# Healthcare-Robotics/assistive-gym

Measured on AMD Instinct MI355X. Metric: env_steps_per_sec, higher is better.
Workload: dtype f32; 1 GPU; FeedingJaco-v1, 4096 lockstep envs per MI355X, random-policy rollout, 5 simulation steps per env step, 50 PGS sweeps; envs_per_gpu=4096, global_envs=4096, reset_pool=256, reset=pool, parallelism=env-sharded x1, obs_allgather=False

## Files before the change

__graft_entry__.py:

```python
import os
import subprocess
import sys

ROOT = os.path.dirname(os.path.abspath(__file__))
if ROOT not in sys.path:
    sys.path.insert(0, ROOT)


def build():
    from assistive_gym_amd.build import build as build_lib
    build_lib(force=True)
    build_lib(out=os.path.join(ROOT, 'assistive_gym_amd', 'lib', 'variants', 'lvs.so'), extra=('-DAGX_PGS_LV=3',), only=['FEEDING'])
    build_lib(out=os.path.join(ROOT, 'assistive_gym_amd', 'lib', 'variants', 'solo.so'), extra=('-DAGX_SOLVE_PAIR=0',), only=['FEEDING'])
    build_lib(out=os.path.join(ROOT, 'assistive_gym_amd', 'lib', 'variants', 'scan4.so'), extra=('-DAGX_GJK_SCAN_WIDE=0', '-DAGX_GJK_SCAN_ONE=0'), only=['FEEDING'])
    build_lib(out=os.path.join(ROOT, 'assistive_gym_amd', 'lib', 'variants', 'finishgjk.so'), extra=('-DAGX_FINISH_SPILL_GJK',), only=['FEEDING'])
    build_lib(out=os.path.join(ROOT, 'assistive_gym_amd', 'lib', 'variants', 'faceplain.so'), extra=('-DAGX_FACE_PLAIN',), only=['FEEDING', 'FEEDING_M'])
    subprocess.check_call(['make', '-C', os.path.join(ROOT, 'oracle')], stdout=subprocess.DEVNULL)
    if os.path.isdir('/root/reference/assistive_gym/envs/assets'):
        from assistive_gym_amd.model import compiler
        compiler.main()
    import assistive_gym_amd
    from assistive_gym_amd import libagx
    L = libagx.load()
    missing = [e for e in libagx.EXPORTS if not hasattr(L, e)]
    assert not missing, missing


def smoke():
    import numpy as np
    sys.path.insert(0, os.path.join(ROOT, 'tests'))
    from assistive_gym_amd import libagx
    from assistive_gym_amd.blob import ModelBlob
    from assistive_gym_amd.vec_env import build_reset_pool
    from oracle_lib import Oracle
    libagx.check(libagx.load().agx_selftest(0), 'agx_selftest')
    n = 64
    for model in ('feeding_jaco', 'bed_bathing_sawyer'):
        blob = ModelBlob.load(model)
        states = build_reset_pool(blob, n, seed=1001)
        st = libagx.Stepper(blob, n)
        st.set_state(states)
        actions = np.random.RandomState(0).uniform(-1, 1, (n, blob.act_dim)).astype(np.float32)
        obs, rew, done, info = st.step_host(actions)
        o = Oracle(blob)
        worst = 0.0
        for i in range(8):
            o_obs, o_rew, _, o_info = o.step(states[i].copy(), actions[i])
            worst = max(worst, float(np.abs(obs[i] - o_obs).max()), abs(float(rew[i]) - o_rew))
        assert np.isfinite(obs).all() and np.isfinite(rew).all()
        assert worst < 1e-3, (model, worst)
        print('smoke ok: 64 %s envs stepped on the GPU (%s kernels), max |obs, reward| deviation from the oracle %.2e' % (model, st.variant(), worst))
        st.close()


if __name__ == '__main__':
    build()
    if len(sys.argv) > 1 and sys.argv[1] == 'smoke':
        smoke()
```

assistive_gym_amd/csrc/agx_collide.h:

```cpp
#pragma once

namespace agx {

struct Cand { v3 pa, pb, n; float dist, gap; };
constexpr float GJK_FAR_MARGIN = 1e-4f;

AGX_DEV void make_shape(const Ctx& c, int col, v3 shift, gjk_shape& s) {
  s.n = CLI(c, col, AGX_C_NVERT);
  s.v = c.bf + c.o_vert + 3 * CLI(c, col, AGX_C_VOFF);
  v3 p; body_xf(c, CLI(c, col, AGX_C_BODY), s.R, p);
  s.p = p - shift; s.box = false;
  s.c = mul(s.R, mk3(CLF(c, col, AGX_C_AABB_C), CLF(c, col, AGX_C_AABB_C + 1), CLF(c, col, AGX_C_AABB_C + 2))) + s.p;
}
AGX_DEV bool narrowphase(const Ctx& c, int ca, int cb, float limit, Cand& out, bool has) {
  const float* AB = c.lds + L_ARENA;
  gjk_shape sa, sb;
  sa.v = nullptr; sa.n = 0; sa.box = false; sa.c = mk3(0.f, 0.f, 0.f); sb.v = nullptr; sb.n = 0; sb.box = false; sb.c = sa.c;
  v3 shift = mk3(0.f, 0.f, 0.f);
  float ra = 0.f, rb = 0.f;
  bool ok = has;
  if (has) {
    shift = mk3(0.5f * (AB[ABS * ca] + AB[ABS * ca + 3]), 0.5f * (AB[ABS * ca + 1] + AB[ABS * ca + 4]), 0.5f * (AB[ABS * ca + 2] + AB[ABS * ca + 5]));
    make_shape(c, ca, shift, sa); make_shape(c, cb, shift, sb);
    if (CLI(c, cb, AGX_C_BODY) == AGX_BODY_WORLD && sb.n == 8 && (CLI(c, cb, AGX_C_TAG) == AGX_TAG_TABLE || CLI(c, cb, AGX_C_TAG) == AGX_TAG_PLANE)) {
      sb.box = true;
      float lo[3], hi[3];
      for (int k = 0; k < 3; k++) {
        lo[k] = fmaxf(AB[ABS * cb + k], AB[ABS * ca + k] - AGX_BOX_CLIP); hi[k] = fminf(AB[ABS * cb + 3 + k], AB[ABS * ca + 3 + k] + AGX_BOX_CLIP);
        if (hi[k] < lo[k]) ok = false;
      }
      sb.lo = mk3(lo[0], lo[1], lo[2]) - shift; sb.hi = mk3(hi[0], hi[1], hi[2]) - shift; sb.c = 0.5f * (sb.lo + sb.hi);
    }
    ra = CLF(c, ca, AGX_C_RADIUS); rb = CLF(c, cb, AGX_C_RADIUS);
  }
  float d; v3 pa, pb, n;
  const bool pen = gjk_distance(sa, sb, PRM(c, AGX_P_GJK_TOL), (int)PRM(c, AGX_P_GJK_MAXIT), limit + ra + rb + GJK_FAR_MARGIN, ok, d, pa, pb);
  if (!ok) return false;
  if (!pen) {
    if (d - ra - rb >= limit) return false;
    n = (1.0f / d) * (pa - pb);
  } else {
    float depth; gjk_penetration(sa, sb, c.bf + c.o_dirs, c.bi[AGX_H_NDIR], depth, n, pa, pb);
    d = -depth;
  }
  out.pa = pa - ra * n + shift; out.pb = pb + rb * n + shift; out.n = n; out.dist = d - ra - rb;
  return true;
}
AGX_DEV float pair_mu(const Ctx& c, int ca, int cb) {
  float plane_mu = c.lds[L_ST + c.s_env + AGX_E_PLANE_FRICTION];
  float mua = CLI(c, ca, AGX_C_TAG) == AGX_TAG_PLANE ? plane_mu : CLF(c, ca, AGX_C_FRICTION);
  float mub = CLI(c, cb, AGX_C_TAG) == AGX_TAG_PLANE ? plane_mu : CLF(c, cb, AGX_C_FRICTION);
  return mua * mub;
}
AGX_DEV void emit_contact(Ctx& c, int slot, int ca, int cb, const Cand& k) {
  float* o = c.gcon + CON_STRIDE * slot; int* oi = (int*)o;
  oi[C_CA] = ca; oi[C_CB] = cb; oi[C_BA] = CLI(c, ca, AGX_C_BODY); oi[C_BB] = CLI(c, cb, AGX_C_BODY);
  st3(o + C_PA, k.pa); st3(o + C_PB, k.pb); st3(o + C_N, k.n); o[C_DIST] = k.dist; o[C_MU] = pair_mu(c, ca, cb); o[C_LAM] = 0.f;
}
constexpr int CAND_STRIDE = 8;
constexpr int TW_WORDS = 6 * (MAX_DOF + MAX_FREE);
constexpr int WL_FIT = (ARENA_WORDS - ABS * MAX_COLL - TW_WORDS) / (1 + CAND_STRIDE);
constexpr int WL_MAX = WL_FIT < 200 ? WL_FIT : 200;
constexpr int A_WL = ABS * MAX_COLL;
constexpr int WL_KEY_MASK = ~((511 << 9) | (3 << 24));
constexpr int A_CAND = A_WL + WL_MAX;
constexpr int A_TW = A_CAND + WL_MAX * CAND_STRIDE;
static_assert(A_TW + TW_WORDS <= ARENA_WORDS, "collision workspace exceeds the arena");
static_assert(MAX_COLL <= 512, "collider indices are packed in 9 bits");
constexpr bool LIST_BYTES = MAX_COLL <= 256;
constexpr int LIST_TAIL = LIST_BYTES ? 8 : 16;
constexpr int WL_CAP = WL_MAX - LIST_TAIL;
template <bool B> struct ListIndex { typedef unsigned short type; };
template <> struct ListIndex<true> { typedef uint8_t type; };
typedef ListIndex<LIST_BYTES>::type list_t;
static_assert(WL_CAP >= 128, "a flush of at least two full passes");

AGX_DEV void emit_from_cand(Ctx& c, int slot, int idx) {
  const float* L = c.lds; const int pr = c.ldsi[L_ARENA + A_WL + idx]; const float* cd = L + L_ARENA + A_CAND + CAND_STRIDE * idx;
  Cand k; k.gap = cd[0]; k.pa = ld3(cd + 1); k.n = ld3(cd + 4); k.dist = cd[7]; k.pb = k.pa - k.dist * k.n;
  emit_contact(c, slot, pr & 511, (pr >> 9) & 511, k);
}
AGX_DEV bool face_box(const Ctx& c, int cb) {
  return CLI(c, cb, AGX_C_BODY) == AGX_BODY_WORLD && CLI(c, cb, AGX_C_NVERT) == 8 && (CLI(c, cb, AGX_C_TAG) == AGX_TAG_TABLE || CLI(c, cb, AGX_C_TAG) == AGX_TAG_PLANE);
}
AGX_DEV bool face_point(const Ctx& c, int ca, int cb, int e, v3 p0, Cand& out) {
  const float* AB = c.lds + L_ARENA;
  const int n = CLI(c, ca, AGX_C_NVERT);
  const float* V = c.bf + c.o_vert + 3 * CLI(c, ca, AGX_C_VOFF);
  m3 R; v3 p; body_xf(c, CLI(c, ca, AGX_C_BODY), R, p);
  const float x0 = AB[ABS * cb], y0 = AB[ABS * cb + 1], x1 = AB[ABS * cb + 3], y1 = AB[ABS * cb + 4], top = AB[ABS * cb + 5];
  float zmin = 3.0e38f;
  for (int v = 0; v < n; v++) { const v3 w = mul(R, mk3(V[3 * v], V[3 * v + 1], V[3 * v + 2])) + p; if (w.x >= x0 && w.x <= x1 && w.y >= y0 && w.y <= y1 && w.z < zmin) zmin = w.z; }
  float cx[1 + AGX_FACE_EXTRA], cy[1 + AGX_FACE_EXTRA];
  cx[0] = p0.x; cy[0] = p0.y;
#pragma unroll
  for (int q = 1; q <= AGX_FACE_EXTRA; q++) { cx[q] = 0.f; cy[q] = 0.f; }
  v3 pick = mk3(0.f, 0.f, 0.f);
  if (e == 0) {
    bool found = false;
    for (int v = 0; v < n && !found; v++) {
      const v3 w = mul(R, mk3(V[3 * v], V[3 * v + 1], V[3 * v + 2])) + p;
      if (w.x >= x0 && w.x <= x1 && w.y >= y0 && w.y <= y1 && w.z <= zmin + AGX_FACE_BAND) { pick = w; found = true; }
    }
    if (!found) return false;
  }
#pragma unroll
  for (int q = 1; q <= AGX_FACE_EXTRA; q++) {
    if (q > e) break;
    int bi = -1; float bd = AGX_FACE_SPREAD * AGX_FACE_SPREAD; v3 bw = mk3(0.f, 0.f, 0.f);
    for (int v = 0; v < n; v++) {
      const v3 w = mul(R, mk3(V[3 * v], V[3 * v + 1], V[3 * v + 2])) + p;
      if (!(w.x >= x0 && w.x <= x1 && w.y >= y0 && w.y <= y1) || w.z > zmin + AGX_FACE_BAND) continue;
      float dmin = 3.0e38f;
#pragma unroll
      for (int k = 0; k <= AGX_FACE_EXTRA; k++) if (k < q) { const float dx = w.x - cx[k], dy = w.y - cy[k]; dmin = fminf(dmin, dx * dx + dy * dy); }
      if (dmin > bd) { bd = dmin; bi = v; bw = w; }
    }
    if (bi < 0) return false;
    cx[q] = bw.x; cy[q] = bw.y; pick = bw;
  }
  const float ra = CLF(c, ca, AGX_C_RADIUS);
  out.n = mk3(0.f, 0.f, 1.f); out.pa = mk3(pick.x, pick.y, pick.z - ra); out.pb = mk3(pick.x, pick.y, top); out.dist = pick.z - ra - top;
  return true;
}
#ifdef AGX_FACE_PLAIN
#undef AGX_FACE
#define AGX_FACE 0
#endif
#ifndef AGX_FACE
#define AGX_FACE 2
#endif
#if AGX_FACE < 0 || AGX_FACE > 2
#error "AGX_FACE: 0, 1 or 2"
#endif
constexpr float FACE_PROOF_GUARD = 1e-4f, FACE_PROOF_GUARD_LIM = 1e-5f;

#if AGX_FACE
AGX_DEV bool face_point_wide(const Ctx& c, int ca, int cb, int e, v3 p0, float& zmin, Cand& out) {
  const float* AB = c.lds + L_ARENA;
  const int n = CLI(c, ca, AGX_C_NVERT), last = n - 1;
  const float* V = c.bf + c.o_vert + 3 * CLI(c, ca, AGX_C_VOFF);
  m3 R; v3 p; body_xf(c, CLI(c, ca, AGX_C_BODY), R, p);
  const float x0 = AB[ABS * cb], y0 = AB[ABS * cb + 1], x1 = AB[ABS * cb + 3], y1 = AB[ABS * cb + 4], top = AB[ABS * cb + 5];
#define FACE_LDV(j, kk) const int i##j = (kk) < last ? (kk) : last; const float vx##j = V[3 * i##j], vy##j = V[3 * i##j + 1], vz##j = V[3 * i##j + 2];
#define FACE_LD8(k) FACE_LDV(0, k) FACE_LDV(1, k + 1) FACE_LDV(2, k + 2) FACE_LDV(3, k + 3) FACE_LDV(4, k + 4) FACE_LDV(5, k + 5) FACE_LDV(6, k + 6) FACE_LDV(7, k + 7)
#define FACE_W(j) const v3 w = mul(R, mk3(vx##j, vy##j, vz##j)) + p; const bool in = w.x >= x0 && w.x <= x1 && w.y >= y0 && w.y <= y1;
#define FACE_ALL8(F) F(0) F(1) F(2) F(3) F(4) F(5) F(6) F(7)
#define FACE_FRESH(i) (mul(R, mk3(V[3 * (i)], V[3 * (i) + 1], V[3 * (i) + 2])) + p)
  float cx[1 + AGX_FACE_EXTRA], cy[1 + AGX_FACE_EXTRA];
  cx[0] = p0.x; cy[0] = p0.y;
#pragma unroll
  for (int q = 1; q <= AGX_FACE_EXTRA; q++) { cx[q] = 0.f; cy[q] = 0.f; }
  v3 pick = mk3(0.f, 0.f, 0.f);
  if (e == 0) {
    int iz = -1; float zm = 3.0e38f;
#define FACE_ZMIN(j) { FACE_W(j) const bool t = in && w.z < zm; zm = t ? w.z : zm; iz = t ? i##j : iz; }
    for (int k = 0; k < n; k += 8) { FACE_LD8(k) FACE_ALL8(FACE_ZMIN) }
#undef FACE_ZMIN
    zmin = 3.0e38f;
    if (iz < 0) return false;
    zmin = FACE_FRESH(iz).z;
    int first = -1;
#define FACE_BAND(j) { FACE_W(j) const bool t = first < 0 && in && w.z <= zmin + AGX_FACE_BAND; first = t ? i##j : first; }
    for (int k = 0; k < n && first < 0; k += 8) { FACE_LD8(k) FACE_ALL8(FACE_BAND) }
#undef FACE_BAND
    if (first < 0) return false;
    pick = FACE_FRESH(first);
  }
#pragma unroll
  for (int q = 1; q <= AGX_FACE_EXTRA; q++) {
    if (q > e) break;
    int bi = -1; float bd = AGX_FACE_SPREAD * AGX_FACE_SPREAD;
#define FACE_FAR(j) { FACE_W(j) float dmin = 3.0e38f; \
      _Pragma("unroll") for (int kk = 0; kk <= AGX_FACE_EXTRA; kk++) if (kk < q) { const float dx = w.x - cx[kk], dy = w.y - cy[kk]; dmin = fminf(dmin, dx * dx + dy * dy); } \
      const bool t = in && !(w.z > zmin + AGX_FACE_BAND) && dmin > bd; bd = t ? dmin : bd; bi = t ? i##j : bi; }
    for (int k = 0; k < n; k += 8) { FACE_LD8(k) FACE_ALL8(FACE_FAR) }
#undef FACE_FAR
    if (bi < 0) return false;
    const v3 bw = FACE_FRESH(bi);
    cx[q] = bw.x; cy[q] = bw.y; pick = bw;
  }
#undef FACE_LDV
#undef FACE_LD8
#undef FACE_W
#undef FACE_ALL8
#undef FACE_FRESH
  const float ra = CLF(c, ca, AGX_C_RADIUS);
  out.n = mk3(0.f, 0.f, 1.f); out.pa = mk3(pick.x, pick.y, pick.z - ra); out.pb = mk3(pick.x, pick.y, top); out.dist = pick.z - ra - top;
  return true;
}
#endif
struct CollideState { int ncon, near_mask, overflow, maxc, nqpt; };
struct GroupRegs { int a0, a1, b0, b1, flags, keep; float alo[3], ahi[3], blo[3], bhi[3]; };
AGX_DEV float body_wmag(const Ctx& c, int code) {
  if (code >= 0 && code < AGX_BODY_ROBOT_BASE) return c.lds[L_WMAG + code];
  if (code >= AGX_BODY_FREE0 && code < AGX_BODY_HUMAN0) return c.lds[L_WMAG + MAX_DOF + (code - AGX_BODY_FREE0)];
  return 0.f;
}
AGX_DEV void body_twist(const Ctx& c, int code, v3& w, v3& v) {
  int slot = -1;
  if (code >= 0 && code < AGX_BODY_ROBOT_BASE) slot = code;
  else if (code >= AGX_BODY_FREE0 && code < AGX_BODY_HUMAN0) slot = MAX_DOF + (code - AGX_BODY_FREE0);
  if (slot < 0) { w = mk3(0.f, 0.f, 0.f); v = w; return; }
  const float* T = c.lds + L_ARENA + A_TW + 6 * slot;
  w = ld3(T); v = ld3(T + 3);
}
AGX_DEV float rel_travel(const Ctx& c, int a, int b) {
  const float* AB = c.lds + L_ARENA;
#ifdef AGX_NO_REL_TRAVEL
  return AB[ABS * a + 6] + AB[ABS * b + 6];
#endif
  v3 wa, va, wb, vb;
  body_twist(c, CLI(c, a, AGX_C_BODY), wa, va); body_twist(c, CLI(c, b, AGX_C_BODY), wb, vb);
  const bool sa = CLI(c, a, AGX_C_NVERT) == 1, sb = CLI(c, b, AGX_C_NVERT) == 1;
  const int e = (!sa && sb) ? b : a;
  const v3 lo = ld3(AB + ABS * e), hi = ld3(AB + ABS * e + 3);
  const v3 ce = 0.5f * (lo + hi), d = hi - lo;
  const v3 dw = wa - wb;
  const v3 u = (va - vb) + cross(dw, ce - ld3(c.lds + L_MISC + M_REF));
  const float rot = (sa || sb) ? 0.f : sqrtf(dot(dw, dw)) * 0.5f * sqrtf(dot(d, d));
  const float t = 1.001f * (sqrtf(dot(u, u)) + rot) * c.dt + 1e-6f;
  return fminf(t, AB[ABS * a + 6] + AB[ABS * b + 6]);
}
AGX_DEV bool sphere_box_apart(const Ctx& c, int x, int y, float reach) {
  const float* AB = c.lds + L_ARENA;
  const v3 cx = mk3(0.5f * (AB[ABS * x] + AB[ABS * x + 3]), 0.5f * (AB[ABS * x + 1] + AB[ABS * x + 4]), 0.5f * (AB[ABS * x + 2] + AB[ABS * x + 5]));
  const v3 hx = mk3(CLF(c, x, AGX_C_AABB_H), CLF(c, x, AGX_C_AABB_H + 1), CLF(c, x, AGX_C_AABB_H + 2));
  const float rx = sqrtf(dot(hx, hx)) + CLF(c, x, AGX_C_RADIUS);
  m3 R; v3 p; body_xf(c, CLI(c, y, AGX_C_BODY), R, p);
  const v3 pl = tmul(R, cx - p) - mk3(CLF(c, y, AGX_C_AABB_C), CLF(c, y, AGX_C_AABB_C + 1), CLF(c, y, AGX_C_AABB_C + 2));
  const float dx = fmaxf(fabsf(pl.x) - CLF(c, y, AGX_C_AABB_H), 0.f), dy = fmaxf(fabsf(pl.y) - CLF(c, y, AGX_C_AABB_H + 1), 0.f),
              dz = fmaxf(fabsf(pl.z) - CLF(c, y, AGX_C_AABB_H + 2), 0.f);
  const float lb = sqrtf(dx * dx + dy * dy + dz * dz) - rx - CLF(c, y, AGX_C_RADIUS);
  return lb > reach;
}

AGX_DEV void collide_flush(Ctx& c, int wn, CollideState& cs, float brk, float slack, const GroupRegs& G) {
  float* L = c.lds; int* WL = c.ldsi + L_ARENA + A_WL; float* CD = L + L_ARENA + A_CAND; const int lane = c.lane;
  const float* AB = L + L_ARENA;
  const int food0 = c.bi[AGX_H_FOOD0];
  if (wn == 0) return;
  wave_sync();
  long long ct0 = c.timing ? wave_clock() : 0;
  if (c.timing) { c.tm[13] += wn; c.tm[14] += (wn + 63) / 64; }
  bool any_manifold_query = false;
  for (int base = 0; base < wn; base += 64) {
    const int i = base + lane; const bool has = i < wn;
    Cand k; k.gap = 3.0e38f; bool near = false; int a = 0, g = 0;
    int b = 0, sub = 0;
    float lim = brk;
    if (has) {
      const int pr = WL[i]; a = pr & 511; b = (pr >> 9) & 511; g = (pr >> 18) & 63; sub = (pr >> 24) & 3;
      if (!(GRI(c, g, AGX_G_FLAGS) & (2 | 64))) lim = fminf(brk, slack + rel_travel(c, a, b) + 1e-5f);
    }
    k.n = mk3(0.f, 0.f, 0.f); k.pa = k.n; k.pb = k.n; k.dist = 0.f;
#if AGX_FACE
    bool proven = false;
    if (has && sub == 0) {
      float* cd = CD + CAND_STRIDE * i; float state = 0.f;
      if (face_box(c, b) && CLI(c, a, AGX_C_NVERT) >= 2) {
        Cand k0; k0.pa = k.pa; k0.dist = 0.f; float zmin;
        const bool first = face_point_wide(c, a, b, 0, k.pa, zmin, k0);
        st3(cd + 1, k0.pa); cd[7] = k0.dist;
#pragma unroll
        for (int q = 1; q <= AGX_FACE_EXTRA; q++) if (i + q < wn) CD[CAND_STRIDE * (i + q)] = zmin;
        state = first ? 1.f : 0.f;
#if AGX_FACE >= 2
        const float* Aa = AB + ABS * a; const float* Bb = AB + ABS * b; const float top = Bb[5], dcore = zmin - top;
        proven = first && Aa[0] >= Bb[0] + FACE_PROOF_GUARD && Aa[3] <= Bb[3] - FACE_PROOF_GUARD && Aa[1] >= Bb[1] + FACE_PROOF_GUARD && Aa[4] <= Bb[4] - FACE_PROOF_GUARD &&
                 Aa[0] <= Aa[3] && Aa[1] <= Aa[4] && Aa[2] - AGX_BOX_CLIP <= top && Aa[5] + AGX_BOX_CLIP >= top && Bb[2] <= top &&
                 dcore > FACE_PROOF_GUARD && dcore - CLF(c, a, AGX_C_RADIUS) - CLF(c, b, AGX_C_RADIUS) < lim - FACE_PROOF_GUARD_LIM;
        if (proven) state = 2.f;
#endif
      }
      cd[0] = state;
    }
    bool hit = narrowphase(c, a, b, lim, k, has && sub == 0 && !proven);
    if (has && sub == 0) {
      const float* cd = CD + CAND_STRIDE * i; const float state = cd[0];
      if (state == 2.f || (state == 1.f && hit && k.n.z > 0.999f)) {
        hit = true; k.n = mk3(0.f, 0.f, 1.f); k.pa = ld3(cd + 1); k.pb = mk3(k.pa.x, k.pa.y, AB[ABS * b + 5]); k.dist = cd[7];
      }
    }
#else
    bool hit = narrowphase(c, a, b, lim, k, has && sub == 0);
    if (has && sub == 0 && hit && k.n.z > 0.999f && face_box(c, b) && CLI(c, a, AGX_C_NVERT) >= 2) { Cand k0; k0.gap = k.gap; if (face_point(c, a, b, 0, k.pa, k0)) k = k0; }
#endif
    if (wave_any(has && sub > 0)) {
      if (has && sub == 0) { float* cd = CD + CAND_STRIDE * i; st3(cd + 1, k.pa); st3(cd + 4, k.n); }
      wave_sync();
      if (has && sub > 0) {
        const float* sd = CD + CAND_STRIDE * (i - sub);
#if AGX_FACE
        float zmin = CD[CAND_STRIDE * i];
        hit = sd[6] > 0.999f && face_point_wide(c, a, b, sub, ld3(sd + 1), zmin, k) && k.dist < brk;
#else
        hit = sd[6] > 0.999f && face_point(c, a, b, sub, ld3(sd + 1), k) && k.dist < brk;
#endif
      }
    }
    if (has) {
      if (hit) {
        near = true;
        v3 vr = point_velocity(c, CLI(c, a, AGX_C_BODY), k.pa) - point_velocity(c, CLI(c, b, AGX_C_BODY), k.pb);
        float pg = k.dist + dot(vr, k.n) * c.dt;
        if (pg < ((GRI(c, g, AGX_G_FLAGS) & 64) ? brk : slack)) k.gap = pg;
      }
      float* cd = CD + CAND_STRIDE * i;
      cd[0] = k.gap; st3(cd + 1, k.pa); st3(cd + 4, k.n); cd[7] = k.dist;
    }
    if constexpr (TASK == AGX_TASK_FEEDING) {
      const bool mq = has && near && (GRI(c, g, AGX_G_FLAGS) & 2) && CLI(c, a, AGX_C_TAG) == AGX_TAG_FOOD;
      if (wave_any(mq)) { any_manifold_query = true; for (int f = 0; f < c.nfood; f++) if (wave_any(mq && CLI(c, a, AGX_C_BODY) - AGX_BODY_FREE0 - food0 == f)) cs.near_mask |= 1 << f; }
    }
    if constexpr (TASK != AGX_TASK_FEEDING) {
      const bool qp = has && near && (GRI(c, g, AGX_G_FLAGS) & 2) && CLI(c, a, AGX_C_TAG) == AGX_TAG_TOOL && (TKI(c, AGX_T_PAD_LINK) >> (CLI(c, a, AGX_C_LINK) + 1) & 1) &&
                      CLI(c, b, AGX_C_TAG) == AGX_TAG_HUMAN;
      const uint64_t qm = wave_ballot(qp);
      const int slot = cs.nqpt + wave_rank(qm);
      if (qp && slot < MAX_QPT) { float* o = c.gqpt + QPT_STRIDE * slot; st3(o, k.pb); ((int*)o)[3] = CLI(c, b, AGX_C_LINK); }
      cs.nqpt += popc64(qm);
    }
  }
  (void)any_manifold_query;
  wave_sync();
  if (c.timing) { long long t = wave_clock(); c.tm[11] += t - ct0; ct0 = t; }
  int* SEL = c.ldsi + L_ARENA + A_CAND + CAND_STRIDE * WL_CAP;
  const int ncon0 = cs.ncon;
  int cur = 0;
  while (cur < wn) {
    const int key = WL[cur] & WL_KEY_MASK;
    const int g = (key >> 18) & 63, keep = wave_bcast_i(G.keep, g);
    const int i0 = cur + lane, i1 = cur + 64 + lane;
    const bool s0 = i0 < wn && (WL[i0 < wn ? i0 : 0] & WL_KEY_MASK) == key, s1 = i1 < wn && (WL[i1 < wn ? i1 : 0] & WL_KEY_MASK) == key;
    const uint64_t b0 = wave_ballot(s0), b1 = wave_ballot(s1);
    const int len0 = (~b0) ? ffs64(~b0) : 64;
    const int len = len0 < 64 ? len0 : 64 + ((~b1) ? ffs64(~b1) : 64);
    const bool in0 = lane < len, in1 = 64 + lane < len;
    float g0 = in0 ? CD[CAND_STRIDE * i0] : 3.0e38f, g1 = in1 ? CD[CAND_STRIDE * i1] : 3.0e38f;
    if (keep == 0) {
      for (int pass = 0; pass < 2; pass++) {
        const bool has = (pass ? g1 : g0) < 1.0e38f;
        const uint64_t m = wave_ballot(has);
        int cnt = popc64(m); const int slot = cs.ncon + wave_rank(m);
        if (has && slot < cs.maxc) SEL[slot - ncon0] = pass ? i1 : i0;
        int room = cs.maxc - cs.ncon; if (room < 0) room = 0;
        if (cnt > room) { cs.overflow += cnt - room; cnt = room; }
        cs.ncon += cnt;
      }
    } else {
      for (int q = 0; q < keep; q++) {
        const float mg = wave_min(fminf(g0, g1));
        if (mg > 1.0e38f) break;
        const uint64_t m0 = wave_ballot(g0 == mg);
        int slot1 = 0, win;
        if (m0) win = ffs64(m0); else { win = ffs64(wave_ballot(g1 == mg)); slot1 = 1; }
        if (cs.ncon < cs.maxc) { if (lane == win) SEL[cs.ncon - ncon0] = slot1 ? i1 : i0; cs.ncon++; } else cs.overflow++;
        if (lane == win) { if (slot1) g1 = 3.0e38f; else g0 = 3.0e38f; }
      }
    }
    cur += len;
  }
  wave_sync();
  if (ncon0 + lane < cs.ncon) emit_from_cand(c, ncon0 + lane, SEL[lane]);
  wave_sync();
  if (c.timing) { long long t = wave_clock(); c.tm[12] += t - ct0; }
}

AGX_DEV int collide_sweep(Ctx& c, int g, int aa, int ab, int b0, int b1, int gflags, float mg, int wn, int rep, const GroupRegs& G) {
  const float* AB = c.lds + L_ARENA; int* WL = c.ldsi + L_ARENA + A_WL; const int lane = c.lane;
  const bool same = gflags & 1, no_adjacent = gflags & 4;
  float ulo[2][3], uhi[2][3];
  for (int q = 0; q < 3; q++) { ulo[0][q] = wave_bcast(G.blo[q], g); uhi[0][q] = wave_bcast(G.bhi[q], g); ulo[1][q] = wave_bcast(G.alo[q], g); uhi[1][q] = wave_bcast(G.ahi[q], g); }
  list_t* LIST = (list_t*)(c.ldsi + L_ARENA + A_CAND + CAND_STRIDE * WL_CAP);
  int nlive[2] = {0, 0};
  for (int side = 0; side < 2; side++) {
    const int r0 = side == 0 ? aa : b0, r1 = side == 0 ? ab : b1;
    for (int base = r0; base < r1; base += 64) {
      const int x = base + lane; bool ok = x < r1;
      if (ok) for (int q = 0; q < 3; q++) if (AB[ABS * x + q] > uhi[side][q] + mg || ulo[side][q] > AB[ABS * x + 3 + q] + mg) ok = false;
      const uint64_t m = wave_ballot(ok);
      if (ok) LIST[128 * side + nlive[side] + wave_rank(m)] = (list_t)x;
      nlive[side] += popc64(m);
    }
  }
  const int na_live = nlive[0], nb = nlive[1];
  wave_sync();
  const int npairs = na_live * nb * rep;
  for (int base = 0; base < npairs; base += 64) {
    const int p = base + lane; bool ok = p < npairs;
    const int pq = ok ? p / rep : 0, sub = ok ? p - pq * rep : 0;
    const int ai = pq / nb; const int a = LIST[ai], b = LIST[128 + pq - ai * nb];
    ok = ok && (!same || b > a) && (sub == 0 || (face_box(c, b) && CLI(c, a, AGX_C_NVERT) >= 2));
    if (ok && no_adjacent) {
      const int la = CLI(c, a, AGX_C_BODY), lb = CLI(c, b, AGX_C_BODY);
      if (la == lb) ok = false;
      else if (la >= 0 && la < AGX_BODY_ROBOT_BASE && lb >= 0 && lb < AGX_BODY_ROBOT_BASE && (RBI(c, la, AGX_R_PARENT) == lb || RBI(c, lb, AGX_R_PARENT) == la)) ok = false;
    }
    if (ok) for (int q = 0; q < 3; q++) if (AB[ABS * a + q] > AB[ABS * b + 3 + q] + mg || AB[ABS * b + q] > AB[ABS * a + 3 + q] + mg) ok = false;
    if (ok) { const float reach = mg + rel_travel(c, a, b) + 1e-5f; ok = !sphere_box_apart(c, a, b, reach) && (CLI(c, a, AGX_C_NVERT) == 1 || !sphere_box_apart(c, b, a, reach)); }
    const uint64_t m = wave_ballot(ok);
    const int slot = wn + wave_rank(m);
    if (ok && slot < WL_CAP) WL[slot] = a | (b << 9) | (g << 18) | (sub << 24);
    wn += popc64(m);
  }
  wave_sync();
  return wn;
}

AGX_DEV void collide(Ctx& c) {
  float* L = c.lds; float* AB = L + L_ARENA; const int lane = c.lane;
  const float brk = PRM(c, AGX_P_CONTACT_BREAK), slack = PRM(c, AGX_P_CONTACT_SLACK);
  CollideState cs; cs.ncon = 0; cs.near_mask = 0; cs.overflow = 0; cs.nqpt = 0;
  cs.maxc = (int)PRM(c, AGX_P_MAX_CONTACTS); if (cs.maxc > MAX_CON) cs.maxc = MAX_CON;
  long long ct0 = c.timing ? wave_clock() : 0, ct1;
#define AGX_CTICK(k) if (c.timing) { ct1 = wave_clock(); c.tm[k] += ct1 - ct0; ct0 = ct1; }
  if (lane < MAX_DOF + MAX_FREE) {
    v3 w = mk3(0, 0, 0), v = w;
    if (lane < MAX_DOF) { if (lane < c.ndof) for (int d = lane; d >= 0; d = RBI(c, d, AGX_R_PARENT)) { const float qd = L[L_VEL + d]; w = w + qd * ld3(L + L_S + 6 * d); v = v + qd * ld3(L + L_S + 6 * d + 3); } }
    else if (lane - MAX_DOF < c.nfree) {
      const int fb = lane - MAX_DOF, o = c.ndof + 6 * fb;
      w = ld3(L + L_VEL + o + 3);
      v = ld3(L + L_VEL + o) + cross(w, ld3(L + L_MISC + M_REF) - ld3(L + L_ST + c.s_free + 13 * fb));
    }
    L[L_WMAG + lane] = sqrtf(dot(w, w));
    st3(AB + A_TW + 6 * lane, w); st3(AB + A_TW + 6 * lane + 3, v);
  }
  wave_sync();
  for (int col = lane; col < c.ncoll; col += 64) {
    const int code = CLI(c, col, AGX_C_BODY);
    m3 R; v3 p; body_xf(c, code, R, p);
    v3 cl = mk3(CLF(c, col, AGX_C_AABB_C), CLF(c, col, AGX_C_AABB_C + 1), CLF(c, col, AGX_C_AABB_C + 2));
    v3 hl = mk3(CLF(c, col, AGX_C_AABB_H), CLF(c, col, AGX_C_AABB_H + 1), CLF(c, col, AGX_C_AABB_H + 2));
    v3 cw = mul(R, cl) + p; float r = CLF(c, col, AGX_C_RADIUS);
    v3 vc = point_velocity(c, code, cw);
    const float wmag = body_wmag(c, code);
    const float grow = (sqrtf(dot(vc, vc)) + wmag * (sqrtf(dot(hl, hl)) + r)) * c.dt;
    for (int k = 0; k < 3; k++) {
      float h = fabsf(R.a[3 * k]) * hl.x + fabsf(R.a[3 * k + 1]) * hl.y + fabsf(R.a[3 * k + 2]) * hl.z + r;
      AB[ABS * col + k] = comp(cw, k) - h - grow; AB[ABS * col + 3 + k] = comp(cw, k) + h + grow;
    }
    AB[ABS * col + 6] = grow;
  }
  wave_sync();
  AGX_CTICK(8)
  const int gender = c.ldsi[L_ST + c.s_env + AGX_E_GENDER];
  uint64_t live_groups = 0;
  GroupRegs G; G.a0 = 0; G.a1 = 0; G.b0 = 0; G.b1 = 0; G.flags = 0; G.keep = 0;
  for (int k = 0; k < 3; k++) { G.alo[k] = 0.f; G.ahi[k] = 0.f; G.blo[k] = 0.f; G.bhi[k] = 0.f; }
  {
    const int g = lane; bool live = false;
    if (g < c.ngroup) {
      G.a0 = GRI(c, g, AGX_G_A0); G.a1 = GRI(c, g, AGX_G_A1); G.b0 = GRI(c, g, AGX_G_B0); G.b1 = GRI(c, g, AGX_G_B1);
      if (gender == 1 && GRI(c, g, AGX_G_B0F) >= 0) { G.b0 = GRI(c, g, AGX_G_B0F); G.b1 = GRI(c, g, AGX_G_B1F); }
      G.flags = GRI(c, g, AGX_G_FLAGS); G.keep = GRI(c, g, AGX_G_KEEP);
      const int a0 = G.a0, a1 = G.a1, b0 = G.b0, b1 = G.b1;
      const float mg = (G.flags & (2 | 64)) ? brk : slack;
      const bool wanted = !((G.flags & 8) && gender != 0) && !((G.flags & 16) && gender != 1) &&
                          !((G.flags & 32) && c.nrobot + c.nhdof <= 32 && ((~c.frozen >> c.nrobot) & ((1u << c.nhdof) - 1u)) == 0);
      if (a1 > a0 && b1 > b0 && wanted) {
        float alo[3] = {3.0e38f, 3.0e38f, 3.0e38f}, ahi[3] = {-3.0e38f, -3.0e38f, -3.0e38f}, blo[3] = {3.0e38f, 3.0e38f, 3.0e38f}, bhi[3] = {-3.0e38f, -3.0e38f, -3.0e38f};
        for (int i = a0; i < a1; i++) for (int k = 0; k < 3; k++) { alo[k] = fminf(alo[k], AB[ABS * i + k]); ahi[k] = fmaxf(ahi[k], AB[ABS * i + 3 + k]); }
        for (int i = b0; i < b1; i++) for (int k = 0; k < 3; k++) { blo[k] = fminf(blo[k], AB[ABS * i + k]); bhi[k] = fmaxf(bhi[k], AB[ABS * i + 3 + k]); }
        live = true;
        for (int k = 0; k < 3; k++) if (alo[k] > bhi[k] + mg || blo[k] > ahi[k] + mg) live = false;
        for (int k = 0; k < 3; k++) { G.alo[k] = alo[k]; G.ahi[k] = ahi[k]; G.blo[k] = blo[k]; G.bhi[k] = bhi[k]; }
      }
    }
    live_groups = wave_ballot(live);
  }
  AGX_CTICK(9)
  int wn = 0, g = 0, ab = -1, abatch = 0;
  while (true) {
    while (g < c.ngroup && !(live_groups >> g & 1)) g++;
    if (g >= c.ngroup) {
      if (wn == 0) break;
    } else {
      const int a0 = wave_bcast_i(G.a0, g), a1 = wave_bcast_i(G.a1, g), b0 = wave_bcast_i(G.b0, g), b1 = wave_bcast_i(G.b1, g);
      const int gflags = wave_bcast_i(G.flags, g);
      const float mg = (gflags & (2 | 64)) ? brk : slack;
      const int rep = face_box(c, b0) ? 1 + AGX_FACE_EXTRA : 1;
      const int nb = (b1 - b0) * rep;
      if (ab < 0) { ab = a0; abatch = a1 - a0; }
      const int ae = ab + abatch < a1 ? ab + abatch : a1;
      int wn2 = collide_sweep(c, g, ab, ae, b0, b1, gflags, mg, wn, rep, G);
      AGX_CTICK(10)
      bool fits = wn2 <= WL_CAP;
      if (!fits && wn == 0) {
        const int small = WL_CAP / nb > 0 ? WL_CAP / nb : 1;
        if (abatch > small) { abatch = small; continue; }
        cs.overflow += wn2 - WL_CAP; wn2 = WL_CAP; fits = true;
      }
      if (fits) {
        wn = wn2; ab = ae;
        if (ab >= a1) { g++; ab = -1; }
        if (ab < 0) continue;
      }
    }
    collide_flush(c, wn, cs, brk, slack, G); wn = 0;
    ct0 = c.timing ? wave_clock() : 0;
  }
  c.ncon = cs.ncon; c.near_mask = cs.near_mask; c.overflow = cs.overflow; c.nqpt = cs.nqpt < MAX_QPT ? cs.nqpt : MAX_QPT;
  wave_sync();
#undef AGX_CTICK
}

}
```

Measured before the change: 678,000 env-steps/s.

## Add block-level AABB summaries for group culling and wave-parallel contact selection

Before the group overlap test, each lane folds a block of collider AABBs into a summary box. Group bounding boxes are then built from these block summaries plus the partial blocks at each end, instead of scanning every collider serially per lane. Contact selection is also done across the whole wave at once: segment boundaries, per-candidate ranks and prefix counts come from ballots, replacing the sequential per-key loop, with a fallback to that loop when any run is longer than 128. Both paths are on by default and can be disabled through macros. A separate variant build is added, and a test-only cap on the worklist size is introduced. The new selection code adds quadratic within-segment rank loops and uses more registers.

```diff
diff --git a/__graft_entry__.py b/__graft_entry__.py
--- a/__graft_entry__.py
+++ b/__graft_entry__.py
@@ -15,6 +15,7 @@
     build_lib(out=os.path.join(ROOT, 'assistive_gym_amd', 'lib', 'variants', 'scan4.so'), extra=('-DAGX_GJK_SCAN_WIDE=0', '-DAGX_GJK_SCAN_ONE=0'), only=['FEEDING'])
     build_lib(out=os.path.join(ROOT, 'assistive_gym_amd', 'lib', 'variants', 'finishgjk.so'), extra=('-DAGX_FINISH_SPILL_GJK',), only=['FEEDING'])
     build_lib(out=os.path.join(ROOT, 'assistive_gym_amd', 'lib', 'variants', 'faceplain.so'), extra=('-DAGX_FACE_PLAIN',), only=['FEEDING', 'FEEDING_M'])
+    build_lib(out=os.path.join(ROOT, 'assistive_gym_amd', 'lib', 'variants', 'frontplain.so'), extra=('-DAGX_COLLIDE_FRONT=0',), only=['FEEDING', 'FEEDING_L', 'BED_BATHING'])
     subprocess.check_call(['make', '-C', os.path.join(ROOT, 'oracle')], stdout=subprocess.DEVNULL)
     if os.path.isdir('/root/reference/assistive_gym/envs/assets'):
         from assistive_gym_amd.model import compiler
diff --git a/assistive_gym_amd/csrc/agx_collide.h b/assistive_gym_amd/csrc/agx_collide.h
--- a/assistive_gym_amd/csrc/agx_collide.h
+++ b/assistive_gym_amd/csrc/agx_collide.h
@@ -69,11 +69,29 @@
 static_assert(MAX_COLL <= 512, "collider indices are packed in 9 bits");
 constexpr bool LIST_BYTES = MAX_COLL <= 256;
 constexpr int LIST_TAIL = LIST_BYTES ? 8 : 16;
+#ifdef AGX_WL_TEST_CAP
+constexpr int WL_CAP = AGX_WL_TEST_CAP;
+static_assert(WL_CAP >= 1 && WL_CAP <= WL_MAX - LIST_TAIL, "AGX_WL_TEST_CAP only lowers the cap");
+#else
 constexpr int WL_CAP = WL_MAX - LIST_TAIL;
+static_assert(WL_CAP >= 128, "a flush of at least two full passes");
+static_assert(!(TASK == AGX_TASK_FEEDING && MAX_COLL == 256 && ARENA_WORDS == 3592) || WL_CAP == 174, "the feeding variant: 174 entries make three narrowphase passes instead of four");
+#endif
 template <bool B> struct ListIndex { typedef unsigned short type; };
 template <> struct ListIndex<true> { typedef uint8_t type; };
 typedef ListIndex<LIST_BYTES>::type list_t;
-static_assert(WL_CAP >= 128, "a flush of at least two full passes");
+#ifndef AGX_COLLIDE_FRONT
+#define AGX_COLLIDE_FRONT 1
+#endif
+#if AGX_COLLIDE_FRONT < 0 || AGX_COLLIDE_FRONT > 1
+#error "AGX_COLLIDE_FRONT: 0 or 1"
+#endif
+#ifndef AGX_FRONT_CULL
+#define AGX_FRONT_CULL AGX_COLLIDE_FRONT
+#endif
+#ifndef AGX_FRONT_SELECT
+#define AGX_FRONT_SELECT AGX_COLLIDE_FRONT
+#endif
 
 AGX_DEV void emit_from_cand(Ctx& c, int slot, int idx) {
   const float* L = c.lds; const int pr = c.ldsi[L_ARENA + A_WL + idx]; const float* cd = L + L_ARENA + A_CAND + CAND_STRIDE * idx;
@@ -328,6 +346,51 @@
   int* SEL = c.ldsi + L_ARENA + A_CAND + CAND_STRIDE * WL_CAP;
   const int ncon0 = cs.ncon;
   int cur = 0;
+#if AGX_FRONT_SELECT
+  constexpr int SEL_R = (WL_CAP + 63) / 64;
+  uint64_t SB[SEL_R], QB[SEL_R];
+#pragma unroll
+  for (int r = 0; r < SEL_R; r++) {
+    const int i = 64 * r + lane;
+    SB[r] = wave_ballot(i < wn && (i == 0 || ((WL[i > 0 ? i - 1 : 0] ^ WL[i < wn ? i : 0]) & WL_KEY_MASK) != 0));
+  }
+  int total = 0, seg0[SEL_R], rank[SEL_R]; bool longrun = false;
+#pragma unroll
+  for (int r = 0; r < SEL_R; r++) {
+    const int i = 64 * r + lane; const bool has = i < wn;
+    int s = 0, e = wn;
+#pragma unroll
+    for (int q = 0; q <= r; q++) { const uint64_t m = q < r ? SB[q] : SB[q] & (~0ull >> (63 - lane)); if (m) s = 64 * q + 63 - clz64(m); }
+#pragma unroll
+    for (int q = SEL_R - 1; q >= r; q--) { const uint64_t m = q > r ? SB[q] : (lane < 63 ? SB[q] & (~0ull << (lane + 1)) : 0ull); if (m) e = 64 * q + ffs64(m); }
+    longrun = longrun || (has && e - s > 128);
+    const float gi = has ? CD[CAND_STRIDE * i] : 3.0e38f;
+    const int keep = wave_shfl_i(G.keep, has ? (WL[i] >> 18) & 63 : 0);
+    int rk = 0;
+    if (gi < 1.0e38f) {
+      if (keep == 0) { for (int j = s; j < i; j++) rk += CD[CAND_STRIDE * j] < 1.0e38f ? 1 : 0; }
+      else for (int j = s; j < e; j++) { const float gj = CD[CAND_STRIDE * j]; rk += (gj < gi || (gj == gi && j < i)) ? 1 : 0; }
+    }
+    seg0[r] = s; rank[r] = rk;
+    QB[r] = wave_ballot(gi < 1.0e38f && (keep == 0 || rk < keep));
+    total += popc64(QB[r]);
+  }
+  if (!wave_any(longrun)) {
+#pragma unroll
+    for (int r = 0; r < SEL_R; r++) {
+      if (!(QB[r] >> lane & 1)) continue;
+      int before = 0;
+#pragma unroll
+      for (int q = 0; q <= r; q++) { const int d = seg0[r] - 64 * q; before += d <= 0 ? 0 : popc64(d >= 64 ? QB[q] : QB[q] & ((1ull << d) - 1ull)); }
+      const int slot = ncon0 + before + rank[r];
+      if (slot < cs.maxc) SEL[slot - ncon0] = 64 * r + lane;
+    }
+    int room = cs.maxc - cs.ncon; if (room < 0) room = 0;
+    if (total > room) { cs.overflow += total - room; total = room; }
+    cs.ncon += total;
+    cur = wn;
+  }
+#endif
   while (cur < wn) {
     const int key = WL[cur] & WL_KEY_MASK;
     const int g = (key >> 18) & 63, keep = wave_bcast_i(G.keep, g);
@@ -408,6 +471,17 @@
   return wn;
 }
 
+#if AGX_FRONT_CULL
+AGX_DEV void range_box(const float* AB, int bsh, int r0, int r1, float* lo, float* hi) {
+  int bl0 = (r0 + (1 << bsh) - 1) >> bsh, bl1 = r1 >> bsh;
+  int h1 = bl0 << bsh, t0 = bl1 << bsh;
+  if (bl0 >= bl1) { h1 = r1; t0 = r1; bl1 = bl0; }
+  for (int i = r0; i < h1; i++) for (int k = 0; k < 3; k++) { lo[k] = fminf(lo[k], AB[ABS * i + k]); hi[k] = fmaxf(hi[k], AB[ABS * i + 3 + k]); }
+  for (int b = bl0; b < bl1; b++) for (int k = 0; k < 3; k++) { lo[k] = fminf(lo[k], AB[A_CAND + 6 * b + k]); hi[k] = fmaxf(hi[k], AB[A_CAND + 6 * b + 3 + k]); }
+  for (int i = t0; i < r1; i++) for (int k = 0; k < 3; k++) { lo[k] = fminf(lo[k], AB[ABS * i + k]); hi[k] = fmaxf(hi[k], AB[ABS * i + 3 + k]); }
+}
+#endif
+
 AGX_DEV void collide(Ctx& c) {
   float* L = c.lds; float* AB = L + L_ARENA; const int lane = c.lane;
   const float brk = PRM(c, AGX_P_CONTACT_BREAK), slack = PRM(c, AGX_P_CONTACT_SLACK);
@@ -445,6 +519,16 @@
   wave_sync();
   AGX_CTICK(8)
   const int gender = c.ldsi[L_ST + c.s_env + AGX_E_GENDER];
+#if AGX_FRONT_CULL
+  int bsh = 0; while ((64 << bsh) < c.ncoll) bsh++;
+  {
+    float lo[3] = {3.0e38f, 3.0e38f, 3.0e38f}, hi[3] = {-3.0e38f, -3.0e38f, -3.0e38f};
+    const int i0 = lane << bsh, i1 = i0 + (1 << bsh) < c.ncoll ? i0 + (1 << bsh) : c.ncoll;
+    for (int i = i0; i < i1; i++) for (int k = 0; k < 3; k++) { lo[k] = fminf(lo[k], AB[ABS * i + k]); hi[k] = fmaxf(hi[k], AB[ABS * i + 3 + k]); }
+    for (int k = 0; k < 3; k++) { AB[A_CAND + 6 * lane + k] = lo[k]; AB[A_CAND + 6 * lane + 3 + k] = hi[k]; }
+  }
+  wave_sync();
+#endif
   uint64_t live_groups = 0;
   GroupRegs G; G.a0 = 0; G.a1 = 0; G.b0 = 0; G.b1 = 0; G.flags = 0; G.keep = 0;
   for (int k = 0; k < 3; k++) { G.alo[k] = 0.f; G.ahi[k] = 0.f; G.blo[k] = 0.f; G.bhi[k] = 0.f; }
@@ -460,8 +544,12 @@
                           !((G.flags & 32) && c.nrobot + c.nhdof <= 32 && ((~c.frozen >> c.nrobot) & ((1u << c.nhdof) - 1u)) == 0);
       if (a1 > a0 && b1 > b0 && wanted) {
         float alo[3] = {3.0e38f, 3.0e38f, 3.0e38f}, ahi[3] = {-3.0e38f, -3.0e38f, -3.0e38f}, blo[3] = {3.0e38f, 3.0e38f, 3.0e38f}, bhi[3] = {-3.0e38f, -3.0e38f, -3.0e38f};
+#if AGX_FRONT_CULL
+        range_box(AB, bsh, a0, a1, alo, ahi); range_box(AB, bsh, b0, b1, blo, bhi);
+#else
         for (int i = a0; i < a1; i++) for (int k = 0; k < 3; k++) { alo[k] = fminf(alo[k], AB[ABS * i + k]); ahi[k] = fmaxf(ahi[k], AB[ABS * i + 3 + k]); }
         for (int i = b0; i < b1; i++) for (int k = 0; k < 3; k++) { blo[k] = fminf(blo[k], AB[ABS * i + k]); bhi[k] = fmaxf(bhi[k], AB[ABS * i + 3 + k]); }
+#endif
         live = true;
         for (int k = 0; k < 3; k++) if (alo[k] > bhi[k] + mg || blo[k] > ahi[k] + mg) live = false;
         for (int k = 0; k < 3; k++) { G.alo[k] = alo[k]; G.ahi[k] = ahi[k]; G.blo[k] = blo[k]; G.bhi[k] = bhi[k]; }
```

After: 689,700 env-steps/s (median of 6 runs). 1.02x the previous value.
